# jdapena/distributed_point_functions

Hardware: AMD Instinct MI355X
Metric: DPF leaf evals/sec, full-domain 2^30 uint64 at 1/2/4/8 GPUs; AES blocks/s (higher is better)
Workload: dtype u64

## Files before the change

distributed_point_functions_amd/csrc/kernels/dpf_device.h:

```cpp
#pragma once
#include <hip/hip_runtime.h>
#include <stdint.h>
#include <string.h>

#include "../../../include/dpf_hip.h"
#include "aes_core.h"

namespace {

struct T0Table {
  uint32_t v[256];
};
constexpr T0Table make_t0() {
  T0Table t{};
  for (int i = 0; i < 256; ++i) {
    uint32_t s = dpf_aes::kSbox[i];
    uint32_t s2 = ((s << 1) ^ ((s & 0x80) ? 0x1b : 0)) & 0xff;
    t.v[i] = s2 | (s << 8) | (s << 16) | ((s2 ^ s) << 24);
  }
  return t;
}
__constant__ T0Table c_t0 = make_t0();

struct RoundKeys {
// ... 129 lines not shown
using dpf_aes::Block4;
using u128 = unsigned __int128;

__device__ __forceinline__ u128 block_u128(Block4 h) {
  return ((u128)h.w3 << 96) | ((u128)h.w2 << 64) | ((u128)h.w1 << 32) | h.w0;
}
__device__ __forceinline__ u128 dpf_u128(dpf_block c) { return ((u128)c.high << 64) | c.low; }

struct ExpandParams {
  int64_t num_items;
  int num_levels;
  int k0;
  int S;
  const dpf_block* seeds_in;
  const uint8_t* ctrl_in;
  const dpf_block* cw_seed;
  const uint8_t* cw_left;
  const uint8_t* cw_right;
  char* out;
  RoundKeys rkl, rkr, rkv, rkd;
  int dyn_chunks;
  int ph_end[3];
  int64_t ph_item[3];
  unsigned int* chunk_counter;
  unsigned long long* clock;
};

__device__ __forceinline__ int64_t take_expand_chunk(const ExpandParams& p, int* lds_counter,
                                                     int64_t done, int& k0, int& S) {
  unsigned int c = 0;
  if ((threadIdx.x & 63) == 0)
    c = p.chunk_counter ? __hip_atomic_fetch_add(p.chunk_counter, 1u, __ATOMIC_RELAXED,
                                                 __HIP_MEMORY_SCOPE_AGENT)
                        : (unsigned int)atomicAdd(lds_counter, 1);
  c = __builtin_amdgcn_readfirstlane(c);
  const unsigned int e0 = (unsigned int)p.ph_end[0], e1 = (unsigned int)p.ph_end[1],
                     e2 = (unsigned int)p.ph_end[2];
  if (c >= e2) return done;
  const int j = (c >= e0) + (c >= e1);
  const unsigned int first = j == 0 ? 0u : (j == 1 ? e0 : e1);
  const unsigned int last = j == 0 ? e0 : (j == 1 ? e1 : e2);
  const int64_t item0 = j == 0 ? p.ph_item[0] : (j == 1 ? p.ph_item[1] : p.ph_item[2]);
  const int64_t group = p.chunk_counter ? 0 : (int64_t)blockIdx.x;
  const int64_t chunk = group * (int64_t)(last - first) + (c - first);
  k0 = p.k0 + 2 * j;
  S = p.S - 2 * j;
  return item0 + chunk * 64 + (int64_t)(threadIdx.x & 63);
}

__device__ __forceinline__ int64_t take_chunk(int* counter, int64_t per_wg, int64_t chunks,
                                              int64_t done) {
  int c = 0;
  if ((threadIdx.x & 63) == 0) c = atomicAdd(counter, 1);
  c = __builtin_amdgcn_readfirstlane(c);
  const int64_t g = (int64_t)blockIdx.x * per_wg + c;
  return c < per_wg && g < chunks ? g * 64 + (int64_t)(threadIdx.x & 63) : done;
}

struct ItemLoop {
  int* counter;
  int64_t per_wg, chunks, done;
  __device__ __forceinline__ int64_t first() const {
    return per_wg ? take_chunk(counter, per_wg, chunks, done)
                  : blockIdx.x * (int64_t)blockDim.x + threadIdx.x;
  }
  __device__ __forceinline__ int64_t next(int64_t u) const {
    return per_wg ? take_chunk(counter, per_wg, chunks, done)
                  : u + (int64_t)gridDim.x * blockDim.x;
  }
// ... 889 lines not shown
```

distributed_point_functions_amd/csrc/kernels/dpf_expand_plan.hip:

```cpp
#include <stdint.h>

#include "../../../include/dpf_hip.h"
#include "dpf_runtime.h"

namespace dpf_rt {

int choose_subtree_depth(int64_t num_starts, int num_levels) {
  const int S = num_levels < max_subtree_depth() ? num_levels : max_subtree_depth();
#if defined(DPF_FORCE_S)
  if (num_levels >= DPF_FORCE_S) return DPF_FORCE_S;
#endif
  double best = -1;
  int best_s = S;
  for (int cand = S; cand >= (num_levels > 0 ? 1 : 0); --cand) {
    const int64_t items = num_starts << (num_levels - cand);
    const int blk = block_for(items);
    const int64_t threads = (int64_t)grid_for(items, blk) * blk;
    const int64_t rounds = (items + threads - 1) / threads;
    const double cost = (double)rounds * (2.0 * (num_levels - cand) + 3.0 * (double)(1ll << cand));
    if (best < 0 || cost < best * 0.999) {
      best = cost;
      best_s = cand;
    }
  }
  return best_s;
}

bool small_shape(int64_t num_starts, int num_levels, int* t, int* D) {
  const int64_t cus = num_cus();
  if (hook_is("DPF_EXPAND_SMALL", '0') || num_levels < 1 || num_starts < 1 || num_starts > cus)
    return false;
  int tt = 0;
  while (tt < num_levels - 1 && (num_starts << (tt + 1)) <= cus) ++tt;
  const int d = num_levels - tt;
  if (d < 1 || d > kSmallMaxD) return false;
  *t = tt;
  *D = d;
  return true;
}

bool top_shape(int64_t num_items, int k0, int* t, int* D) {
  const int64_t starts = num_items >> k0;
  if (hook_is("DPF_EXPAND_TOP", '0') || k0 < 8 || starts > num_cus() ||
      num_items < 4 * (int64_t)num_cus())
    return false;
  int tt = 0;
  while ((starts << tt) < num_cus() && tt < k0 - 1) ++tt;
  if (k0 - tt > kSmallMaxD) tt = k0 - kSmallMaxD;
  if (k0 - tt < 1 || (starts << tt) > INT32_MAX) return false;
  *t = tt;
  *D = k0 - tt;
  return true;
}

static int octet_dynamic_shift(int S) {
  return hook_int("DPF_OCTET_DYNAMIC", S >= 11 ? 4 : 2, 0, 4);
}
int octet_walk_levels() { return hook_int("DPF_OCTET_WALK", 2, 0, 4); }
ChunkPlan plan_chunks(int64_t num_items, int k0, int S, int min_S, int64_t cus, bool sched_ok) {
  ChunkPlan c{};
  const int sh = octet_dynamic_shift(S);
  if (sh <= 0 || S - sh < min_S || k0 + sh > 62 || cus <= 0 || num_items <= 0 ||
      num_items > (INT64_MAX >> (sh + 4)) || (num_items << sh) % (cus * 64) != 0 ||
      (num_items << sh) < 4 * cus * max_block() || (num_items << sh) / 64 > (INT32_MAX >> 4))
    return c;
  c.shift = sh;
  const int big = sched_ok && (num_items << S) / cus >= ((int64_t)1 << 20);
  c.global = hook_int("DPF_OCTET_GLOBAL", big, 0, 1);
  c.groups = c.global ? 1 : cus;
  const int k = k0 + sh, s = S - sh;
  const int64_t coarse = (num_items << sh) / 64;
  const int finer = hook_int("DPF_OCTET_TAPER", big ? 2 : 0, 0, 2);
  const int64_t at = hook_int("DPF_OCTET_TAPER_AT", 2, 1, 16) * cus * (max_block() / 64);
  auto exists = [&](int j) { return j <= finer && s - 2 * j >= min_S && k + 2 * j <= 62; };
  int64_t start[4] = {0, coarse, coarse, coarse};
  if (exists(1)) start[1] = coarse - (coarse < at ? coarse : at);
  if (exists(2)) start[2] = coarse - (coarse - start[1] < (at >> 2) ? coarse - start[1] : (at >> 2));
  for (int j = 0; j < 3; ++j) {
    c.k0[j] = k + 2 * j;
    c.S[j] = s - 2 * j;
    c.chunks[j] = (start[j + 1] - start[j]) << (2 * j);
    c.first_item[j] = (start[j] * 64) << (2 * j);
  }
  return c;
}

void write_plan(const ChunkPlan& c, int64_t* out) {
  for (int i = 0; i < 15; ++i) out[i] = 0;
  out[0] = c.shift;
  if (!c.shift) return;
  out[1] = c.global;
  out[2] = c.groups;
  for (int j = 0; j < 3; ++j) {
    out[3 + 4 * j] = c.chunks[j];
    out[4 + 4 * j] = c.first_item[j];
    out[5 + 4 * j] = c.k0[j];
    out[6 + 4 * j] = c.S[j];
  }
}

}

using namespace dpf_rt;

extern "C" int dpf_hip_octet_schedule(int64_t num_items, int k0, int subtree_depth, int min_depth,
                                      int compute_units, int64_t* out) {
  if (!out) return fail(kInvalidArgument, "NULL pointer");
  if (num_items < 1 || k0 < 0 || subtree_depth < 0 || k0 + subtree_depth > 62 ||
      compute_units < 1)
    return fail(kInvalidArgument, "launch shape out of range");
  write_plan(plan_chunks(num_items, k0, subtree_depth, min_depth, compute_units, true), out);
  return kOk;
}
```

distributed_point_functions_amd/csrc/kernels/dpf_kernels.hip:

```cpp
#include <hip/hip_runtime.h>
#include <stdint.h>
#include <stdlib.h>
#include <string.h>

#include <atomic>
#include <type_traits>
#include <vector>
#include <string>

#include "../../../include/dpf_hip.h"
#include "dpf_device.h"
#include "dpf_dot.h"
#include "dpf_runtime.h"

namespace dpf_rt {
thread_local std::string g_last_error;
thread_local const char* g_last_expand = "";
thread_local int g_last_expand_s = -1;
thread_local int64_t g_last_dynamic_chunks = 0;
std::atomic<unsigned long long*> g_clock_acc{nullptr};

int fail(int code, const std::string& msg) {
  g_last_error = msg;
  return code;
// ... 53 lines not shown
  for (int64_t i = items.first(); i < p.n; i = items.next(i)) {
    Block4 s = load_block(p.seeds_in + i);
    uint32_t t = p.ctrl_in[i] & 1u;
    Block4 path = load_block(p.paths + i);
    for (int j = 0; j < p.num_levels; ++j) {
      uint32_t bit = path_bit(path, p.num_levels - 1 - j);
      path_step(lk, lk.ks.l, lk.ks.d, s, t, bit, lds.cw_seed[j], lds.cw_ctrl[j]);
    }
    store_block(p.seeds_out + i, s);
    p.ctrl_out[i] = (uint8_t)t;
  }
}

template <class Leaf, bool SCHED = false>
__global__ __launch_bounds__(kBlock) DPF_WAVES_ATTR void expand_kernel(ExpandParams p, Leaf leaf) {
  __shared__ LdsImage lds;
  __shared__ int next_chunk;
  leaf.init();
  fill_tables(lds.tab);
  fill_cws(lds, p.cw_seed, p.cw_left, p.cw_right, p.num_levels);
  if (threadIdx.x == 0) next_chunk = 0;
  __syncthreads();
  const LdsLookup lk = make_lookup(lds, KeySet{key_ref(p.rkl), key_ref(p.rkr), key_ref(p.rkv), key_ref(p.rkd)});
  int k0 = p.k0, S = p.S;
  if constexpr (SCHED) ClockStamp::first_begin(p.clock);
  const int64_t nch = (p.num_items + 63) / 64;
  const int64_t end = SCHED ? INT64_MAX : p.num_items;
  auto take = [&]() -> int64_t {
    if constexpr (SCHED) return take_expand_chunk(p, &next_chunk, end, k0, S);
    else return take_chunk(&next_chunk, p.dyn_chunks, nch, p.num_items);
  };
  for (int64_t item = SCHED || p.dyn_chunks ? take()
                                            : blockIdx.x * (int64_t)blockDim.x + threadIdx.x;
       item < end;
       item = SCHED || p.dyn_chunks ? take() : item + (int64_t)gridDim.x * blockDim.x) {
    const int B = S >= 1 ? 1 : 0;
    const int G = S - B;
    const int64_t ngroups = (int64_t)1 << G;
    const int64_t r = item >> k0;
    Block4 s = load_block(p.seeds_in + r);
    uint32_t t = p.ctrl_in[r] & 1u;
    for (int j = 0; j < k0; ++j) {
      uint32_t bit = (uint32_t)((item >> (k0 - 1 - j)) & 1);
      path_step(lk, lk.ks.l, lk.ks.d, s, t, bit, lds.cw_seed[j], lds.cw_ctrl[j]);
    }
    Block4 sib[kGMax];
    uint32_t tb = 0;
    const int64_t leaf_base = item << S;
    for (int64_t g = 0; g < ngroups; ++g) {
      Block4 node = s;
      uint32_t nt = t;
      int ds = 0;
      if (g != 0) {
        ds = G - (int)__builtin_ctzll((unsigned long long)g);
#pragma unroll
        for (int d = 1; d <= kGMax; ++d)
          if (d == ds) { node = sib[d - 1]; nt = (tb >> d) & 1u; }
      }
      for (int d = ds; d < G; ++d) {
        Block4 c0, c1;
        uint32_t t0, t1;
        children_step(lk, lk.ks.l, lk.ks.r, node, nt, lds.cw_seed[k0 + d], lds.cw_ctrl[k0 + d],
                      c0, t0, c1, t1);
#pragma unroll
        for (int e = 1; e <= kGMax; ++e)
          if (e == d + 1) sib[e - 1] = c1;
// ... 63 lines not shown
  }
  leaf.store4(x, first_leaf, out);
}

template <class Leaf> struct OctetStash { static constexpr int value = 2; };
template <> struct OctetStash<SwarLeaf> { static constexpr int value = 1; };

template <class Leaf, bool SCHED = false>
__global__ __launch_bounds__(kBlock) DPF_WAVES_ATTR void expand_octet_kernel(ExpandParams p,
                                                                             Leaf leaf) {
  __shared__ LdsImage lds;
  constexpr int kStash = OctetStash<Leaf>::value;
  __shared__ uint4 stash[kBlock];
  __shared__ uint3 stash2[kStash >= 2 ? kBlock : 1];
  __shared__ int next_chunk;
  static_assert(sizeof(LdsImage) + 16 * kBlock + (kStash >= 2 ? 12 * kBlock : 0) + 16 <= 160 * 1024,
                "LDS over 160 KiB");
  leaf.init();
  fill_tables(lds.tab);
  fill_cws(lds, p.cw_seed, p.cw_left, p.cw_right, p.num_levels);
  if (threadIdx.x == 0) next_chunk = 0;
  __syncthreads();
  const LdsLookup lk = make_lookup(lds, KeySet{key_ref(p.rkl), key_ref(p.rkr), key_ref(p.rkv), key_ref(p.rkd)});
  int k0 = p.k0, S = p.S;
  ClockStamp stamp;
  stamp.begin(p.clock);
  const int lane = (int)(threadIdx.x & 63);
  const int64_t end = SCHED ? INT64_MAX : p.num_items;
  auto take = [&]() -> int64_t {
    if constexpr (SCHED) {
      return take_expand_chunk(p, &next_chunk, end, k0, S);
    } else {
      int c = 0;
      if (lane == 0) c = atomicAdd(&next_chunk, 1);
      c = __builtin_amdgcn_readfirstlane(c);
      return c < p.dyn_chunks ? ((int64_t)blockIdx.x * p.dyn_chunks + c) * 64 + lane
                              : p.num_items;
    }
  };
  for (int64_t item = SCHED || p.dyn_chunks ? take()
                                            : blockIdx.x * (int64_t)blockDim.x + threadIdx.x;
       item < end;
       item = SCHED || p.dyn_chunks ? take() : item + (int64_t)gridDim.x * blockDim.x) {
    const int G = S - 3;
    const int64_t ngroups = (int64_t)1 << G;
    const int64_t r = item >> k0;
    Block4 s = load_block(p.seeds_in + r);
    uint32_t t = p.ctrl_in[r] & 1u;
    for (int j = 0; j < k0; ++j) {
      const uint32_t bit = (uint32_t)((item >> (k0 - 1 - j)) & 1);
      path_step(lk, lk.ks.l, lk.ks.d, s, t, bit, lds.cw_seed[j], lds.cw_ctrl[j]);
    }
    Block4 sib[kGMax];
    uint32_t tb = 0;
    const int64_t leaf_base = item << S;
    Block4 next = s;
    for (int64_t g = 0; g < ngroups; ++g) {
      Block4 node = next;
      uint32_t nt = t;
      int ds = 0;
      if (g != 0) {
        ds = G - (int)__builtin_ctzll((unsigned long long)g);
        nt = (tb >> ds) & 1u;
      }
      for (int d = ds; d < G; ++d) {
        Block4 c0, c1;
        uint32_t t0, t1;
        children_step(lk, lk.ks.l, lk.ks.r, node, nt, lds.cw_seed[k0 + d], lds.cw_ctrl[k0 + d],
                      c0, t0, c1, t1);
        sib[d] = c1;
        tb = (tb & ~(1u << (d + 1))) | (t1 << (d + 1));
        node = c0;
        nt = t0;
// ... 121 lines not shown
                     lds.cw_ctrl[lvl], c0, t0, c1, t1);
      quad::hash2(lk, qv, c0, c1);
      const Block4 h0 = quad::gather(c0), h1 = quad::gather(c1);
      if (c == 0) {
        leaf.store(leaf.correct(h0, t0), leaf0 + 2 * q, p.out);
        leaf.store(leaf.correct(h1, t1), leaf0 + 2 * q + 1, p.out);
      }
    }
  } else if (tid < npar) {
    const uint4 v = nodes[tid];
    Block4 c0, c1;
    uint32_t t0, t1;
    children_step(lk, lk.ks.l, lk.ks.r, Block4{v.x, v.y, v.z, v.w}, tbits[tid], lds.cw_seed[lvl],
                  lds.cw_ctrl[lvl], c0, t0, c1, t1);
    leaf.emit2(lk, lk.ks.v, c0, t0, c1, t1, leaf0 + 2 * tid, p.out);
  }
  if constexpr (HasFinish<Leaf>::value) leaf.finish();
}

struct SeedLeaf {
  dpf_block* seeds;
  uint8_t* ctrl;
  unsigned int* counter;
  __device__ __forceinline__ void init() const {
    if (counter != nullptr && blockIdx.x == 0 && threadIdx.x == 0) *counter = 0u;
  }
  __device__ __forceinline__ void emit2(const LdsLookup&, KeyRef, Block4 s0, uint32_t t0, Block4 s1,
                                        uint32_t t1, int64_t first, char*) const {
    store_block(seeds + first, s0);
    store_block(seeds + first + 1, s1);
    ctrl[first] = (uint8_t)t0;
    ctrl[first + 1] = (uint8_t)t1;
  }
};

__global__ void count_out_of_range_kernel(int64_t n, const dpf_block* __restrict__ pts, int log,
                                          unsigned long long* __restrict__ bad) {
  unsigned long long c = 0;
  for (int64_t i = blockIdx.x * (int64_t)blockDim.x + threadIdx.x; i < n;
       i += (int64_t)gridDim.x * blockDim.x) {
    const dpf_block b = pts[i];
    bool out;
    if (log >= 128) out = false;
    else if (log >= 64) out = (b.high >> (log - 64)) != 0;
    else out = b.high != 0 || (b.low >> log) != 0;
    c += out ? 1 : 0;
  }
  for (int off = 32; off > 0; off >>= 1) c += __shfl_down(c, off, 64);
// ... 131 lines not shown
  int t = 0, D = 0;
  const int64_t starts = p0.num_items >> p0.k0;
  if (!small_shape(starts, p0.num_levels, &t, &D)) return false;
  ExpandParams p = p0;
  p.k0 = t;
  p.S = D;
  p.num_items = starts << t;
  static const std::string name = std::string("small/") + leaf_name<Leaf>();
  g_last_expand = name.c_str();
  g_last_expand_s = D;
  hipLaunchKernelGGL((expand_small_kernel<Leaf>), dim3((unsigned)p.num_items), dim3(kBlock), 0, s,
                     p, leaf);
  return true;
}


struct TopScratch {
  void* mem = nullptr;
  hipStream_t s = nullptr;
  ~TopScratch() {
    if (mem) (void)hipFreeAsync(mem, s);
  }
};
int expand_top(ExpandParams& p, hipStream_t s, TopScratch& scratch,
               unsigned int** counter = nullptr) {
  const int64_t starts = p.num_items >> p.k0;
  int t = 0, D = 0;
  if (!top_shape(p.num_items, p.k0, &t, &D)) return kOk;
  static const bool pool_kept = [] {
    int dev = 0;
    hipMemPool_t pool;
    if (hipGetDevice(&dev) != hipSuccess || hipDeviceGetDefaultMemPool(&pool, dev) != hipSuccess)
      return false;
    uint64_t keep = UINT64_MAX;
    return hipMemPoolSetAttribute(pool, hipMemPoolAttrReleaseThreshold, &keep) == hipSuccess;
  }();
  (void)pool_kept;
  const size_t items = (size_t)p.num_items;
  void* mem = nullptr;
  const size_t roots = (items * (sizeof(dpf_block) + 1) + 127) / 128 * 128;
  HIP_TRY(hipMallocAsync(&mem, roots + (counter ? 128 : 0), s));
  scratch.mem = mem;
  scratch.s = s;
  SeedLeaf leaf{static_cast<dpf_block*>(mem),
                static_cast<uint8_t*>(mem) + items * sizeof(dpf_block),
                counter ? reinterpret_cast<unsigned int*>(static_cast<char*>(mem) + roots)
                        : nullptr};
  if (counter) *counter = leaf.counter;
  ExpandParams q = p;
  q.k0 = t;
  q.S = D;
  q.num_levels = p.k0;
  q.num_items = starts << t;
  q.clock = nullptr;
  hipLaunchKernelGGL((expand_small_kernel<SeedLeaf>), dim3((unsigned)q.num_items), dim3(kBlock), 0,
                     s, q, leaf);
  HIP_TRY(hipGetLastError());
  p.seeds_in = leaf.seeds;
  p.ctrl_in = leaf.ctrl;
  p.cw_seed += p.k0;
  p.cw_left += p.k0;
  p.cw_right += p.k0;
  p.num_levels = p.S;
  p.k0 = 0;
  return kOk;
}

thread_local ChunkPlan g_last_plan{};
int subtree_shape(ExpandParams& p, int min_S, hipStream_t s, TopScratch& top, int* grid,
                  int* blk, bool sched_ok) {
  p.dyn_chunks = 0;
  p.chunk_counter = nullptr;
  g_last_plan = ChunkPlan{};
  const int64_t cus = num_cus();
  const ChunkPlan plan = plan_chunks(p.num_items, p.k0, p.S, min_S, cus, sched_ok);
  if (const int sh = plan.shift) {
    ExpandParams q = p;
    q.S -= sh;
    q.k0 += sh;
    q.num_items <<= sh;
    q.dyn_chunks = (int)(q.num_items / (cus * 64));
    int64_t taken = 0;
    for (int j = 0; j < 3; ++j) {
      taken += plan.chunks[j] / plan.groups;
      q.ph_end[j] = (int)taken;
      q.ph_item[j] = plan.first_item[j];
    }
    unsigned int* counter = nullptr;
    unsigned int** want_counter = plan.global ? &counter : nullptr;
    const int w = octet_walk_levels();
    int up = w > 0 && q.k0 - w >= 8 ? w : 0;
    ExpandParams t;
    for (;; up = 0) {
      t = q;
      t.k0 = q.k0 - up;
      t.S = q.S + up;
      t.num_items = q.num_items >> up;
      if (int st = expand_top(t, s, top, want_counter)) return st;
      if (t.k0 == 0 || up == 0) break;
    }
    if (t.k0 == 0) {
      q.chunk_counter = counter;
      q.seeds_in = t.seeds_in;
      q.ctrl_in = t.ctrl_in;
      q.cw_seed = t.cw_seed;
      q.cw_left = t.cw_left;
      q.cw_right = t.cw_right;
      q.num_levels = q.S + up;
      q.k0 = up;
      p = q;
      g_last_plan = plan;
      *grid = (int)cus;
      *blk = kBlock;
      return kOk;
    }
  }
  if (int st = expand_top(p, s, top)) return st;
  *blk = block_for(p.num_items);
  *grid = grid_for(p.num_items, *blk);
  return kOk;
}
template <class Leaf, bool OCTET> struct SchedDefault { static constexpr bool value = true; };
template <> struct SchedDefault<SwarLeaf, true> { static constexpr bool value = false; };
template <> struct SchedDefault<Mod32Leaf<kMod32MaxLeaves>, false> {
  static constexpr bool value = false;
};
bool has_schedule(const ExpandParams& p) {
  return p.dyn_chunks && (p.chunk_counter || p.ph_end[0] != p.ph_end[2]);
}
template <class Leaf> struct HasOctet : std::false_type {};
template <int BITS, bool XOR> struct HasOctet<FastIntLeaf<BITS, XOR>> : std::true_type {};
template <int BITS, bool XOR> struct HasOctet<DotLeaf<BITS, XOR>> : std::true_type {};
template <> struct HasOctet<SwarLeaf> : std::true_type {};
template <> struct HasOctet<Mod32Leaf<2>> : std::true_type {};
// ... 131 lines not shown
  auto sec = [&](unsigned long long t) { return (double)(int64_t)(t - t0) * 1e-8; };
  double lo = 0, hi = 0, sum = 0;
  int n = 0;
  for (int i = 0; i < kProbeWorkgroups; ++i) {
    if (!h[kProbeWords + i]) continue;
    const double t = sec(h[kProbeWords + i]);
    lo = n ? (t < lo ? t : lo) : t;
    hi = n ? (t > hi ? t : hi) : t;
    sum += t;
    ++n;
  }
  out[0] = sec(~h[kProbeFirstExit]);
  out[1] = sec(h[kProbeLastExit]);
  out[2] = lo;
  out[3] = hi;
  out[4] = n ? sum / n : 0.0;
  out[5] = n;
  return kOk;
}

int dpf_hip_last_expand_schedule(int64_t* out) {
  if (!out) return fail(kInvalidArgument, "NULL pointer");
  dpf_rt::write_plan(g_last_plan, out);
  return kOk;
}

int dpf_hip_clock_probe_read(double* clock_ghz, int64_t* workgroups, double* mean_workgroup_s) {
  unsigned long long* acc = dpf_rt::g_clock_acc.load();
  if (!acc) return fail(kFailedPrecondition, "clock probe is off (dpf_hip_clock_probe(1))");
  unsigned long long h[4] = {0, 0, 0, 0};
  HIP_TRY(hipDeviceSynchronize());
  HIP_TRY(hipMemcpy(h, acc, sizeof(h), hipMemcpyDeviceToHost));
  HIP_TRY(hipMemset(acc, 0, kProbeBytes));
  HIP_TRY(hipDeviceSynchronize());
  if (clock_ghz) *clock_ghz = h[1] ? (double)h[0] / (double)h[1] * 0.1 : 0.0;
  if (workgroups) *workgroups = (int64_t)h[2];
  if (mean_workgroup_s) *mean_workgroup_s = h[2] ? (double)h[1] / (double)h[2] * 1e-8 : 0.0;
  return kOk;
}

int dpf_hip_packed_element_size(const dpf_value_desc* desc) {
  if (!desc) return -1;
  return packed_size(desc);
}

int dpf_hip_hash(int64_t n, const dpf_block* in, const dpf_aes_key* key, dpf_block* out,
// ... 230 lines not shown
```

distributed_point_functions_amd/csrc/kernels/dpf_runtime.h:

```cpp
#pragma once
#include <hip/hip_runtime.h>
#include <stdint.h>
#include <stdlib.h>

#include <string>
#include <type_traits>

#include "../../../include/dpf_hip.h"

namespace dpf_rt {

constexpr int kOk = 0, kInvalidArgument = 3, kResourceExhausted = 8, kFailedPrecondition = 9,
              kUnimplemented = 12, kInternal = 13;

int fail(int code, const std::string& msg);
int hip_fail(hipError_t e, const char* what);

inline bool hook_is(const char* name, char c) {
  const char* v = getenv(name);
  return v && v[0] == c;
}
inline bool hook_set(const char* name) { return getenv(name) != nullptr; }
inline long long hook_long(const char* name, long long dflt) {
  const char* v = getenv(name);
// ... 13 lines not shown
int grid_for(int64_t work_items, int block);
struct LaunchShape {
  int block, grid;
  int64_t dyn_per_wg;
};
LaunchShape chunked_shape(int64_t items, const char* hook);
template <class F>
auto with_bits(int bits, F&& f) {
  switch (bits) {
    case 8: return f(std::integral_constant<int, 8>{});
    case 16: return f(std::integral_constant<int, 16>{});
    case 32: return f(std::integral_constant<int, 32>{});
    case 64: return f(std::integral_constant<int, 64>{});
    default: return f(std::integral_constant<int, 128>{});
  }
}
struct ChunkPlan {
  int shift;
  int global;
  int64_t groups;
  int k0[3], S[3];
  int64_t chunks[3], first_item[3];
};
ChunkPlan plan_chunks(int64_t num_items, int k0, int S, int min_S, int64_t cus, bool sched_ok);
void write_plan(const ChunkPlan& c, int64_t* out);
constexpr int kSmallMaxD = 11;
int choose_subtree_depth(int64_t num_starts, int num_levels);
bool small_shape(int64_t num_starts, int num_levels, int* t, int* D);
bool top_shape(int64_t num_items, int k0, int* t, int* D);
int octet_walk_levels();
int validate_desc(const dpf_value_desc* d);
int packed_size(const dpf_value_desc* d);
bool fast_int(const dpf_value_desc* d);

extern thread_local const char* g_last_dot;
int dot_type(const dpf_value_desc* d, int* words, int* xor_type);
int launch_dot_fold(int row_words, int xor_type, int accumulate, const void* workspace, void* out,
                    hipStream_t s);

constexpr int kHHSketchMaxRows = 2;
int launch_sketch_slot_weights(int64_t n, int64_t count, const int64_t* src_offset, int rows,
                               const uint32_t* weights, const uint32_t mod[2], uint32_t* out,
                               hipStream_t s);
int launch_hh_level(const dpf_prefix_batch_args& a, int b, hipStream_t s);
int launch_hh_keys(const dpf_prefix_batch_args& a, int b, hipStream_t s);

template <class Params>
void set_batch_tables(Params* p, const dpf_prefix_batch_args& a) {
  p->num_keys = a.num_keys;
  p->num_starts = a.num_starts;
  p->cw_stride = a.cw_stride;
  p->seeds_in = a.seeds_in;
// ... 23 lines not shown
```

distributed_point_functions_amd/hip_abi.py:

```python
from __future__ import annotations

import ctypes
import os
import re
from typing import Optional, Sequence

import numpy as np

_HERE = os.path.dirname(os.path.abspath(__file__))
LIB_PATH = os.environ.get("DPF_HIP_LIB") or os.path.join(_HERE, "lib", "libdpf_hip.so")
HEADER = os.path.join(os.path.dirname(_HERE), "include", "dpf_hip.h")
MAX_LEAVES = 16
LEAF_INT, LEAF_INTMODN, LEAF_XOR = 0, 1, 2
MASK64 = (1 << 64) - 1

_lib = None


class DpfHipError(RuntimeError):
    def __init__(self, code: int, msg: str):
        super().__init__(f"[{code}] {msg}")
        self.code = code


# ... 65 lines not shown
        L.dpf_hip_last_points_kernel.restype = ctypes.c_char_p
        L.dpf_hip_last_points_kernel.argtypes = []
        L.dpf_hip_hash.argtypes = [I64, P, P, P, P]
        L.dpf_hip_eval_paths.argtypes = [I64, I, P, P, P, P, P, P, P, P, P, P, P]
        L.dpf_hip_expand.argtypes = [I64, P, P, I, P, P, P, P, P, P, P, I, P, I, P, P]
        L.dpf_hip_eval_points.argtypes = [I64, I64, I, P, P, P, P, P, P, P, P, P, P, P, P, P, P,
                                          P, P]
        L.dpf_hip_gather.argtypes = [I64, I64, I, P, P, P, P]
        L.dpf_hip_sum_shares_u64.argtypes = [I64, I64, I, I, P, P, P]
        L.dpf_hip_packed_element_size.argtypes = [P]
        L.dpf_hip_event_create.argtypes = [ctypes.POINTER(ctypes.c_void_p)]
        L.dpf_hip_event_destroy.argtypes = [P]
        L.dpf_hip_event_record.argtypes = [P, P]
        L.dpf_hip_event_elapsed_ms.argtypes = [P, P, ctypes.POINTER(ctypes.c_float)]
        L.dpf_hip_stream_sync.argtypes = [P]
        L.dpf_hip_clock_probe.argtypes = [I]
        L.dpf_hip_clock_probe_read.argtypes = [ctypes.POINTER(ctypes.c_double),
                                               ctypes.POINTER(ctypes.c_int64),
                                               ctypes.POINTER(ctypes.c_double)]
        for name, types in (("dpf_hip_clock_probe_exits", [ctypes.POINTER(ctypes.c_double)]),
                            ("dpf_hip_octet_schedule",
                             [I64, I, I, I, I, ctypes.POINTER(ctypes.c_int64)]),
                            ("dpf_hip_last_expand_schedule", [ctypes.POINTER(ctypes.c_int64)]),
                            ("dpf_hip_last_dynamic_chunks", [ctypes.POINTER(ctypes.c_int64)]),
                            ("dpf_hip_mic_eval_batch",
                             [I64, I, P, P, P, P, P, I, P, P, I, P, I] + [P] * 11),
                            ("dpf_hip_expand_dot",
                             [I64, P, P, I, P, P, P, P, P, P, P, I, P, I, P, I, P, P, P]),
                            ("dpf_hip_dot_rows", [I64, I, P, P, P, I, P, P, P]),
                            ("dpf_hip_expand_dot_workspace_bytes", [P, I]),
                            ("dpf_hip_expand_dot_fused", [P, I]),
                            ("dpf_hip_last_dot_kernel", []),
                            ("dpf_hip_select_rows", [I64, I, I, P, I64, P, I, P, P, P]),
                            ("dpf_hip_select_workspace_bytes", [I, I]),
                            ("dpf_hip_last_select_shape", [ctypes.POINTER(ctypes.c_int64)]),
                            ("dpf_hip_dot_rows_batch", [I64, I, I, P, P, I64, P, I, P, P, P]),
                            ("dpf_hip_dot_rows_batch_workspace_bytes", [P, I, I]),
                            ("dpf_hip_last_dot_batch_shape", [ctypes.POINTER(ctypes.c_int64)]),
                            ("dpf_hip_sketch_rows", [I64, I64, P, P, I, I, P, P, P]),
                            ("dpf_hip_sketch_supported", [P]),
                            ("dpf_hip_gen_keys_supported", [P]),
                            ("dpf_hip_gen_key_batch",
                             [I64, I, I, P, P, P, P, P, P, P, I, I, P, P, P, P, P, P, P, P]),
                            ("dpf_hip_prefix_batch_sketch_fused", [P, I, I, I, I, I, I]),
                            ("dpf_hip_sketch_slot_weights", [I64, I64, P, P, I, P, P, P]),
                            ("dpf_hip_dcf_expand_supported", [P, I, P]),
# ... 208 lines not shown
def clock_probe_exits() -> dict:
    out = (ctypes.c_double * 6)()
    check(load().dpf_hip_clock_probe_exits(out))
    ms = [v * 1e3 for v in out[:5]]
    return {"first_exit_ms": ms[0], "last_exit_ms": ms[1], "workgroup_last_exit_min_ms": ms[2],
            "workgroup_last_exit_max_ms": ms[3], "workgroup_last_exit_mean_ms": ms[4],
            "workgroups": int(out[5])}


def octet_schedule(num_items: int, k0: int, subtree_depth: int, min_depth: int,
                   compute_units: int) -> dict:
    out = (ctypes.c_int64 * 15)()
    check(load().dpf_hip_octet_schedule(num_items, k0, subtree_depth, min_depth, compute_units,
                                        out))
    return _plan(out)


def last_expand_schedule() -> dict:
    out = (ctypes.c_int64 * 15)()
    check(load().dpf_hip_last_expand_schedule(out))
    return _plan(out)


def _plan(out) -> dict:
    phases = [{"chunks": out[3 + 4 * j], "first_item": out[4 + 4 * j], "k0": out[5 + 4 * j],
               "depth": out[6 + 4 * j]} for j in range(3) if out[3 + 4 * j]]
    return {"shift": out[0], "global": bool(out[1]), "counters": out[2], "phases": phases}


def check(st: int):
    if st != 0:
        raise DpfHipError(st, load().dpf_hip_last_error().decode())


def aes_key(k: int) -> AesKey:
    a = AesKey()
    for i, b in enumerate((k & ((1 << 128) - 1)).to_bytes(16, "little")):
        a.bytes[i] = b
    return a


def value_desc(leaves: Sequence[tuple], direct: bool, elements_per_block: int,
               blocks_needed: int) -> ValueDesc:
    d = ValueDesc()
    d.num_leaves = len(leaves)
    d.direct = 1 if direct else 0
# ... 278 lines not shown
```

include/dpf_hip.h:

```cpp
#ifndef DPF_HIP_H_
#define DPF_HIP_H_

#include <stddef.h>
#include <stdint.h>

#ifdef __cplusplus
extern "C" {
#endif

#define DPF_HIP_ABI_VERSION 2
#define DPF_MAX_LEAVES 16

typedef struct dpf_block {
  uint64_t low;
  uint64_t high;
} dpf_block;

typedef struct dpf_aes_key {
  uint8_t bytes[16];
} dpf_aes_key;

enum dpf_leaf_kind { DPF_LEAF_INT = 0, DPF_LEAF_INTMODN = 1, DPF_LEAF_XOR = 2 };

typedef struct dpf_value_desc {
// ... 78 lines not shown
int dpf_hip_select_workspace_bytes(int record_words, int num_queries);
int dpf_hip_last_select_shape(int64_t* out3);

#define DPF_HIP_DOT_BATCH_MAX_QUERIES 64
int dpf_hip_dot_rows_batch(int64_t num_rows, int record_words, int num_queries,
                           const dpf_value_desc* desc, const void* y, int64_t y_stride_bytes,
                           const void* db, int accumulate, void* workspace, void* out,
                           void* stream);
int dpf_hip_dot_rows_batch_workspace_bytes(const dpf_value_desc* desc, int record_words,
                                           int num_queries);
int dpf_hip_last_dot_batch_shape(int64_t* out3);

const char* dpf_hip_last_expand_kernel(int* subtree_depth);

int dpf_hip_clock_probe(int on);
int dpf_hip_clock_probe_read(double* clock_ghz, int64_t* workgroups, double* mean_workgroup_s);

int dpf_hip_clock_probe_exits(double* out);

int dpf_hip_octet_schedule(int64_t num_items, int k0, int subtree_depth, int min_depth,
                           int compute_units, int64_t* out);

int dpf_hip_last_expand_schedule(int64_t* out);

const char* dpf_hip_last_batch_kernel(void);

const char* dpf_hip_last_points_kernel(void);

int dpf_hip_last_dynamic_chunks(int64_t* per_wg);

int dpf_hip_eval_points(int64_t num_points, int64_t points_per_key, int num_levels,
                        const dpf_block* key_seed, const uint8_t* party,
                        const dpf_block* seeds_in, const uint8_t* control_in,
                        const dpf_block* tree_index, const int32_t* block_index,
                        const dpf_block* cw_seed, const uint8_t* cw_left,
                        const uint8_t* cw_right, const dpf_aes_key* key_left,
                        const dpf_aes_key* key_right, const dpf_aes_key* key_value,
                        const dpf_value_desc* desc, const dpf_block* value_correction,
                        void* out, void* stream);

int dpf_hip_eval_points_batch(int64_t num_keys, int64_t points_per_key, int shared_points,
                              int num_levels, int cw_stride, int block_index_bits,
                              const dpf_block* key_seed,
                              const uint8_t* party, const dpf_block* points,
                              const dpf_block* cw_seed, const uint8_t* cw_left,
                              const uint8_t* cw_right, const dpf_aes_key* key_left,
// ... 208 lines not shown
```

Baseline: 74.23 billion.

## Precompute per-chunk subtree roots so scheduled expand skips redundant path walks

Adds a roots plan that expands the top of the tree down to every chunk's root depth in a few extra kernel launches and stores those seeds in scratch memory. The scheduled expand kernels then load each item's root directly instead of walking k0 levels of AES path steps per item. Initial chunks are also assigned statically by wave index, with the global counter preset past them, which removes the first atomic. The taper and global thresholds are retuned for the roots path. In exchange it adds scratch allocation, extra launches and more complex planning logic.

```diff
diff --git a/distributed_point_functions_amd/csrc/kernels/dpf_device.h b/distributed_point_functions_amd/csrc/kernels/dpf_device.h
--- a/distributed_point_functions_amd/csrc/kernels/dpf_device.h
+++ b/distributed_point_functions_amd/csrc/kernels/dpf_device.h
@@ -175,17 +175,25 @@
   int dyn_chunks;
   int ph_end[3];
   int64_t ph_item[3];
+  int ph_roots;
+  int64_t ph_root[3];
   unsigned int* chunk_counter;
+  int chunk_first;
   unsigned long long* clock;
 };
 
+template <bool FIRST>
 __device__ __forceinline__ int64_t take_expand_chunk(const ExpandParams& p, int* lds_counter,
-                                                     int64_t done, int& k0, int& S) {
+                                                     int64_t done, int& k0, int& S, int& walk,
+                                                     int64_t& root) {
   unsigned int c = 0;
-  if ((threadIdx.x & 63) == 0)
+  if (FIRST && p.chunk_counter && p.chunk_first) {
+    c = blockIdx.x * (blockDim.x >> 6) + (threadIdx.x >> 6);
+  } else if ((threadIdx.x & 63) == 0) {
     c = p.chunk_counter ? __hip_atomic_fetch_add(p.chunk_counter, 1u, __ATOMIC_RELAXED,
                                                  __HIP_MEMORY_SCOPE_AGENT)
                         : (unsigned int)atomicAdd(lds_counter, 1);
+  }
   c = __builtin_amdgcn_readfirstlane(c);
   const unsigned int e0 = (unsigned int)p.ph_end[0], e1 = (unsigned int)p.ph_end[1],
                      e2 = (unsigned int)p.ph_end[2];
@@ -198,6 +206,8 @@
   const int64_t chunk = group * (int64_t)(last - first) + (c - first);
   k0 = p.k0 + 2 * j;
   S = p.S - 2 * j;
+  walk = p.ph_roots ? 0 : k0;
+  root = j == 0 ? p.ph_root[0] : (j == 1 ? p.ph_root[1] : p.ph_root[2]);
   return item0 + chunk * 64 + (int64_t)(threadIdx.x & 63);
 }
 
diff --git a/distributed_point_functions_amd/csrc/kernels/dpf_expand_plan.hip b/distributed_point_functions_amd/csrc/kernels/dpf_expand_plan.hip
--- a/distributed_point_functions_amd/csrc/kernels/dpf_expand_plan.hip
+++ b/distributed_point_functions_amd/csrc/kernels/dpf_expand_plan.hip
@@ -10,6 +10,7 @@
 #if defined(DPF_FORCE_S)
   if (num_levels >= DPF_FORCE_S) return DPF_FORCE_S;
 #endif
+  if (const int forced = hook_int("DPF_EXPAND_SUBTREE", 0, 0, S); forced >= 1) return forced;
   double best = -1;
   int best_s = S;
   for (int cand = S; cand >= (num_levels > 0 ? 1 : 0); --cand) {
@@ -40,12 +41,14 @@
 }
 
 bool top_shape(int64_t num_items, int k0, int* t, int* D) {
+  return top_shape_for(num_items, k0, num_cus(), t, D);
+}
+bool top_shape_for(int64_t num_items, int k0, int64_t cus, int* t, int* D) {
   const int64_t starts = num_items >> k0;
-  if (hook_is("DPF_EXPAND_TOP", '0') || k0 < 8 || starts > num_cus() ||
-      num_items < 4 * (int64_t)num_cus())
+  if (hook_is("DPF_EXPAND_TOP", '0') || k0 < 8 || starts > cus || num_items < 4 * cus)
     return false;
   int tt = 0;
-  while ((starts << tt) < num_cus() && tt < k0 - 1) ++tt;
+  while ((starts << tt) < cus && tt < k0 - 1) ++tt;
   if (k0 - tt > kSmallMaxD) tt = k0 - kSmallMaxD;
   if (k0 - tt < 1 || (starts << tt) > INT32_MAX) return false;
   *t = tt;
@@ -57,20 +60,25 @@
   return hook_int("DPF_OCTET_DYNAMIC", S >= 11 ? 4 : 2, 0, 4);
 }
 int octet_walk_levels() { return hook_int("DPF_OCTET_WALK", 2, 0, 4); }
-ChunkPlan plan_chunks(int64_t num_items, int k0, int S, int min_S, int64_t cus, bool sched_ok) {
+ChunkPlan plan_chunks(int64_t num_items, int k0, int S, int min_S, int64_t cus, bool sched_ok,
+                      bool item_roots) {
   ChunkPlan c{};
   const int sh = octet_dynamic_shift(S);
+  const int64_t per_thread = hook_int("DPF_OCTET_MIN_PER_THREAD", 4, 0, 4);
   if (sh <= 0 || S - sh < min_S || k0 + sh > 62 || cus <= 0 || num_items <= 0 ||
       num_items > (INT64_MAX >> (sh + 4)) || (num_items << sh) % (cus * 64) != 0 ||
-      (num_items << sh) < 4 * cus * max_block() || (num_items << sh) / 64 > (INT32_MAX >> 4))
+      (num_items << sh) < per_thread * cus * max_block() ||
+      (num_items << sh) / 64 > (INT32_MAX >> 4))
     return c;
   c.shift = sh;
-  const int big = sched_ok && (num_items << S) / cus >= ((int64_t)1 << 20);
+  const int64_t per_cu = (num_items << S) / cus;
+  const int big = sched_ok && per_cu >= ((int64_t)1 << (item_roots ? 19 : 20));
+  const int finer_dflt = !big ? 0 : (per_cu >= ((int64_t)1 << 20) ? 2 : 1);
   c.global = hook_int("DPF_OCTET_GLOBAL", big, 0, 1);
   c.groups = c.global ? 1 : cus;
   const int k = k0 + sh, s = S - sh;
   const int64_t coarse = (num_items << sh) / 64;
-  const int finer = hook_int("DPF_OCTET_TAPER", big ? 2 : 0, 0, 2);
+  const int finer = hook_int("DPF_OCTET_TAPER", finer_dflt, 0, 2);
   const int64_t at = hook_int("DPF_OCTET_TAPER_AT", 2, 1, 16) * cus * (max_block() / 64);
   auto exists = [&](int j) { return j <= finer && s - 2 * j >= min_S && k + 2 * j <= 62; };
   int64_t start[4] = {0, coarse, coarse, coarse};
@@ -83,6 +91,79 @@
     c.first_item[j] = (start[j] * 64) << (2 * j);
   }
   return c;
+}
+
+RootsPlan plan_roots(const ChunkPlan& c, int64_t num_items, int k0, int S, int64_t cus) {
+  RootsPlan r{};
+  if (!c.shift || hook_is("DPF_EXPAND_ROOTS", '0') || hook_set("DPF_OCTET_WALK")) return r;
+  const int64_t starts = num_items >> k0;
+  const int kd = c.k0[0];
+  if (starts < 1 || (starts << k0) != num_items) return r;
+  int d = 8;
+  while (d < kd - 1 && (starts << d) < cus * max_block()) ++d;
+  if (d < kd - max_subtree_depth()) d = kd - max_subtree_depth();
+  int t = 0, D = 0;
+  if (d > kd - 1 || !top_shape_for(starts << d, d, cus, &t, &D)) return r;
+  r.top_depth = d;
+  r.top_nodes = starts << d;
+  for (int j = 0; j < 3; ++j)
+    if (c.chunks[j]) r.stages = j + 1;
+  int64_t base = r.top_nodes;
+  for (int j = 0; j < r.stages; ++j) {
+    RootsPlan::Stage& st = r.st[j];
+    const int64_t all = starts << c.k0[j];
+    st.in_depth = j ? c.k0[j - 1] : d;
+    st.levels = c.k0[j] - st.in_depth;
+    st.out_first = j ? c.first_item[j] : 0;
+    st.out_count = all - st.out_first;
+    st.in_first = st.out_first >> st.levels;
+    st.in_count = st.out_count >> st.levels;
+    st.base = base;
+    base += st.out_count;
+    if ((st.in_first << st.levels) != st.out_first || c.first_item[j] < st.out_first ||
+        c.first_item[j] + c.chunks[j] * 64 > st.out_first + st.out_count ||
+        st.in_count > INT32_MAX)
+      return RootsPlan{};
+  }
+  r.nodes = base;
+  r.bytes = (base * 17 + 127) / 128 * 128 + 128;
+  r.bound = ((num_items << S) * 16) / 8;
+  if (r.bytes > r.bound) return RootsPlan{};
+  r.on = 1;
+  return r;
+}
+
+ChunkPlan plan_for_roots(int64_t num_items, int k0, int S, int min_S, int64_t cus, bool sched_ok,
+                         RootsPlan* roots) {
+  const ChunkPlan c = plan_chunks(num_items, k0, S, min_S, cus, sched_ok, true);
+  *roots = plan_roots(c, num_items, k0, S, cus);
+  if (roots->on) return c;
+  const ChunkPlan w = plan_chunks(num_items, k0, S, min_S, cus, sched_ok, false);
+  *roots = plan_roots(w, num_items, k0, S, cus);
+  return w;
+}
+
+void write_roots_plan(const RootsPlan& r, int64_t* out) {
+  for (int i = 0; i < kRootsPlanWords; ++i) out[i] = 0;
+  out[0] = r.on;
+  if (!r.on) return;
+  out[1] = r.top_depth;
+  out[2] = r.top_nodes;
+  out[3] = r.stages;
+  out[4] = r.nodes;
+  out[5] = r.bytes;
+  out[6] = r.bound;
+  for (int j = 0; j < r.stages; ++j) {
+    const RootsPlan::Stage& st = r.st[j];
+    int64_t* o = out + 8 + 7 * j;
+    o[0] = st.in_depth;
+    o[1] = st.levels;
+    o[2] = st.in_first;
+    o[3] = st.in_count;
+    o[4] = st.out_first;
+    o[5] = st.out_count;
+    o[6] = st.base;
+  }
 }
 
 void write_plan(const ChunkPlan& c, int64_t* out) {
@@ -109,6 +190,18 @@
   if (num_items < 1 || k0 < 0 || subtree_depth < 0 || k0 + subtree_depth > 62 ||
       compute_units < 1)
     return fail(kInvalidArgument, "launch shape out of range");
-  write_plan(plan_chunks(num_items, k0, subtree_depth, min_depth, compute_units, true), out);
+  write_plan(plan_chunks(num_items, k0, subtree_depth, min_depth, compute_units, true, false), out);
   return kOk;
 }
+
+extern "C" int dpf_hip_expand_roots_plan(int64_t num_items, int k0, int subtree_depth,
+                                         int min_depth, int compute_units, int64_t* out) {
+  if (!out) return fail(kInvalidArgument, "NULL pointer");
+  if (num_items < 1 || k0 < 0 || subtree_depth < 0 || k0 + subtree_depth > 62 ||
+      compute_units < 1)
+    return fail(kInvalidArgument, "launch shape out of range");
+  RootsPlan r;
+  (void)plan_for_roots(num_items, k0, subtree_depth, min_depth, compute_units, true, &r);
+  write_roots_plan(r, out);
+  return kOk;
+}
diff --git a/distributed_point_functions_amd/csrc/kernels/dpf_kernels.hip b/distributed_point_functions_amd/csrc/kernels/dpf_kernels.hip
--- a/distributed_point_functions_amd/csrc/kernels/dpf_kernels.hip
+++ b/distributed_point_functions_amd/csrc/kernels/dpf_kernels.hip
@@ -99,26 +99,29 @@
   if (threadIdx.x == 0) next_chunk = 0;
   __syncthreads();
   const LdsLookup lk = make_lookup(lds, KeySet{key_ref(p.rkl), key_ref(p.rkr), key_ref(p.rkv), key_ref(p.rkd)});
-  int k0 = p.k0, S = p.S;
+  int k0 = p.k0, S = p.S, walk = p.k0;
+  int64_t root = 0;
   if constexpr (SCHED) ClockStamp::first_begin(p.clock);
   const int64_t nch = (p.num_items + 63) / 64;
   const int64_t end = SCHED ? INT64_MAX : p.num_items;
-  auto take = [&]() -> int64_t {
-    if constexpr (SCHED) return take_expand_chunk(p, &next_chunk, end, k0, S);
+  auto take = [&](auto first) -> int64_t {
+    if constexpr (SCHED)
+      return take_expand_chunk<decltype(first)::value>(p, &next_chunk, end, k0, S, walk, root);
     else return take_chunk(&next_chunk, p.dyn_chunks, nch, p.num_items);
   };
-  for (int64_t item = SCHED || p.dyn_chunks ? take()
+  for (int64_t item = SCHED || p.dyn_chunks ? take(std::true_type{})
                                             : blockIdx.x * (int64_t)blockDim.x + threadIdx.x;
        item < end;
-       item = SCHED || p.dyn_chunks ? take() : item + (int64_t)gridDim.x * blockDim.x) {
+       item = SCHED || p.dyn_chunks ? take(std::false_type{})
+                                    : item + (int64_t)gridDim.x * blockDim.x) {
     const int B = S >= 1 ? 1 : 0;
     const int G = S - B;
     const int64_t ngroups = (int64_t)1 << G;
-    const int64_t r = item >> k0;
+    const int64_t r = SCHED ? (item >> walk) + root : item >> k0;
     Block4 s = load_block(p.seeds_in + r);
     uint32_t t = p.ctrl_in[r] & 1u;
-    for (int j = 0; j < k0; ++j) {
-      uint32_t bit = (uint32_t)((item >> (k0 - 1 - j)) & 1);
+    for (int j = 0; j < walk; ++j) {
+      uint32_t bit = (uint32_t)((item >> (walk - 1 - j)) & 1);
       path_step(lk, lk.ks.l, lk.ks.d, s, t, bit, lds.cw_seed[j], lds.cw_ctrl[j]);
     }
     Block4 sib[kGMax];
@@ -228,14 +231,15 @@
   if (threadIdx.x == 0) next_chunk = 0;
   __syncthreads();
   const LdsLookup lk = make_lookup(lds, KeySet{key_ref(p.rkl), key_ref(p.rkr), key_ref(p.rkv), key_ref(p.rkd)});
-  int k0 = p.k0, S = p.S;
+  int k0 = p.k0, S = p.S, walk = p.k0;
+  int64_t root = 0;
   ClockStamp stamp;
   stamp.begin(p.clock);
   const int lane = (int)(threadIdx.x & 63);
   const int64_t end = SCHED ? INT64_MAX : p.num_items;
-  auto take = [&]() -> int64_t {
+  auto take = [&](auto first) -> int64_t {
     if constexpr (SCHED) {
-      return take_expand_chunk(p, &next_chunk, end, k0, S);
+      return take_expand_chunk<decltype(first)::value>(p, &next_chunk, end, k0, S, walk, root);
     } else {
       int c = 0;
       if (lane == 0) c = atomicAdd(&next_chunk, 1);
@@ -244,17 +248,18 @@
                               : p.num_items;
     }
   };
-  for (int64_t item = SCHED || p.dyn_chunks ? take()
+  for (int64_t item = SCHED || p.dyn_chunks ? take(std::true_type{})
                                             : blockIdx.x * (int64_t)blockDim.x + threadIdx.x;
        item < end;
-       item = SCHED || p.dyn_chunks ? take() : item + (int64_t)gridDim.x * blockDim.x) {
+       item = SCHED || p.dyn_chunks ? take(std::false_type{})
+                                    : item + (int64_t)gridDim.x * blockDim.x) {
     const int G = S - 3;
     const int64_t ngroups = (int64_t)1 << G;
-    const int64_t r = item >> k0;
+    const int64_t r = SCHED ? (item >> walk) + root : item >> k0;
     Block4 s = load_block(p.seeds_in + r);
     uint32_t t = p.ctrl_in[r] & 1u;
-    for (int j = 0; j < k0; ++j) {
-      const uint32_t bit = (uint32_t)((item >> (k0 - 1 - j)) & 1);
+    for (int j = 0; j < walk; ++j) {
+      const uint32_t bit = (uint32_t)((item >> (walk - 1 - j)) & 1);
       path_step(lk, lk.ks.l, lk.ks.d, s, t, bit, lds.cw_seed[j], lds.cw_ctrl[j]);
     }
     Block4 sib[kGMax];
@@ -422,8 +427,14 @@
   dpf_block* seeds;
   uint8_t* ctrl;
   unsigned int* counter;
+  unsigned int counter_init;
   __device__ __forceinline__ void init() const {
-    if (counter != nullptr && blockIdx.x == 0 && threadIdx.x == 0) *counter = 0u;
+    if (counter != nullptr && blockIdx.x == 0 && threadIdx.x == 0) *counter = counter_init;
+  }
+  __device__ __forceinline__ void emit(const LdsLookup&, KeyRef, Block4 s0, uint32_t t0,
+                                       int64_t first, char*) const {
+    store_block(seeds + first, s0);
+    ctrl[first] = (uint8_t)t0;
   }
   __device__ __forceinline__ void emit2(const LdsLookup&, KeyRef, Block4 s0, uint32_t t0, Block4 s1,
                                         uint32_t t1, int64_t first, char*) const {
@@ -601,11 +612,7 @@
     if (mem) (void)hipFreeAsync(mem, s);
   }
 };
-int expand_top(ExpandParams& p, hipStream_t s, TopScratch& scratch,
-               unsigned int** counter = nullptr) {
-  const int64_t starts = p.num_items >> p.k0;
-  int t = 0, D = 0;
-  if (!top_shape(p.num_items, p.k0, &t, &D)) return kOk;
+void keep_pool() {
   static const bool pool_kept = [] {
     int dev = 0;
     hipMemPool_t pool;
@@ -615,6 +622,13 @@
     return hipMemPoolSetAttribute(pool, hipMemPoolAttrReleaseThreshold, &keep) == hipSuccess;
   }();
   (void)pool_kept;
+}
+int expand_top(ExpandParams& p, hipStream_t s, TopScratch& scratch,
+               unsigned int** counter = nullptr, unsigned int counter_init = 0) {
+  const int64_t starts = p.num_items >> p.k0;
+  int t = 0, D = 0;
+  if (!top_shape(p.num_items, p.k0, &t, &D)) return kOk;
+  keep_pool();
   const size_t items = (size_t)p.num_items;
   void* mem = nullptr;
   const size_t roots = (items * (sizeof(dpf_block) + 1) + 127) / 128 * 128;
@@ -624,7 +638,8 @@
   SeedLeaf leaf{static_cast<dpf_block*>(mem),
                 static_cast<uint8_t*>(mem) + items * sizeof(dpf_block),
                 counter ? reinterpret_cast<unsigned int*>(static_cast<char*>(mem) + roots)
-                        : nullptr};
+                        : nullptr,
+                counter_init};
   if (counter) *counter = leaf.counter;
   ExpandParams q = p;
   q.k0 = t;
@@ -645,14 +660,89 @@
   return kOk;
 }
 
+bool expand_roots(ExpandParams& q, const RootsPlan& rp, hipStream_t s, TopScratch& scratch,
+                  unsigned int** counter, unsigned int counter_init, int* st) {
+  *st = kOk;
+  const int64_t starts = rp.top_nodes >> rp.top_depth;
+  int t = 0, D = 0;
+  if (!top_shape(rp.top_nodes, rp.top_depth, &t, &D)) return false;
+  keep_pool();
+  void* mem = nullptr;
+  if (hipMallocAsync(&mem, (size_t)rp.bytes, s) != hipSuccess) {
+    (void)hipGetLastError();
+    return false;
+  }
+  scratch.mem = mem;
+  scratch.s = s;
+  dpf_block* seeds = static_cast<dpf_block*>(mem);
+  uint8_t* ctrl = static_cast<uint8_t*>(mem) + (size_t)rp.nodes * sizeof(dpf_block);
+  unsigned int* cnt =
+      counter ? reinterpret_cast<unsigned int*>(static_cast<char*>(mem) + rp.bytes - 128) : nullptr;
+  if (counter) *counter = cnt;
+  auto failed = [&](hipError_t e) {
+    if (e != hipSuccess) *st = hip_fail(e, "item roots launch");
+    return e != hipSuccess;
+  };
+  ExpandParams e = q;
+  e.dyn_chunks = 0;
+  e.chunk_counter = nullptr;
+  e.clock = nullptr;
+  e.out = nullptr;
+  e.seeds_in = q.seeds_in;
+  e.k0 = t;
+  e.S = D;
+  e.num_levels = rp.top_depth;
+  e.num_items = starts << t;
+  hipLaunchKernelGGL((expand_small_kernel<SeedLeaf>), dim3((unsigned)e.num_items), dim3(kBlock), 0,
+                     s, e, SeedLeaf{seeds, ctrl, cnt, counter_init});
+  if (failed(hipGetLastError())) return true;
+  int64_t in_base = 0, in_first = 0;
+  for (int j = 0; j < rp.stages; ++j) {
+    const RootsPlan::Stage& g = rp.st[j];
+    e.k0 = 0;
+    e.S = g.levels;
+    e.num_levels = g.levels;
+    e.num_items = g.in_count;
+    e.seeds_in = seeds + in_base + (g.in_first - in_first);
+    e.ctrl_in = ctrl + in_base + (g.in_first - in_first);
+    e.cw_seed = q.cw_seed + g.in_depth;
+    e.cw_left = q.cw_left + g.in_depth;
+    e.cw_right = q.cw_right + g.in_depth;
+    const int blk = block_for(g.in_count);
+    hipLaunchKernelGGL((expand_kernel<SeedLeaf, false>), dim3(grid_for(g.in_count, blk)), dim3(blk),
+                       0, s, e, SeedLeaf{seeds + g.base, ctrl + g.base, nullptr, 0u});
+    if (failed(hipGetLastError())) return true;
+    in_base = g.base;
+    in_first = g.out_first;
+    q.ph_root[j] = (g.base - rp.st[0].base) - g.out_first;
+  }
+  for (int j = rp.stages; j < 3; ++j) q.ph_root[j] = 0;
+  q.ph_roots = 1;
+  q.seeds_in = seeds + rp.st[0].base;
+  q.ctrl_in = ctrl + rp.st[0].base;
+  q.cw_seed += q.k0;
+  q.cw_left += q.k0;
+  q.cw_right += q.k0;
+  q.num_levels = q.S;
+  q.k0 = 0;
+  return true;
+}
+
 thread_local ChunkPlan g_last_plan{};
+thread_local RootsPlan g_last_roots{};
+thread_local int g_last_chunk_first = 0;
 int subtree_shape(ExpandParams& p, int min_S, hipStream_t s, TopScratch& top, int* grid,
                   int* blk, bool sched_ok) {
   p.dyn_chunks = 0;
   p.chunk_counter = nullptr;
+  p.chunk_first = 0;
+  p.ph_roots = 0;
   g_last_plan = ChunkPlan{};
+  g_last_roots = RootsPlan{};
+  g_last_chunk_first = 0;
   const int64_t cus = num_cus();
-  const ChunkPlan plan = plan_chunks(p.num_items, p.k0, p.S, min_S, cus, sched_ok);
+  RootsPlan roots;
+  const ChunkPlan plan = plan_for_roots(p.num_items, p.k0, p.S, min_S, cus, sched_ok, &roots);
   if (const int sh = plan.shift) {
     ExpandParams q = p;
     q.S -= sh;
@@ -667,6 +757,25 @@
     }
     unsigned int* counter = nullptr;
     unsigned int** want_counter = plan.global ? &counter : nullptr;
+    const int chunk_first = plan.global && !hook_is("DPF_EXPAND_ROOTS", '0');
+    const unsigned int counter_init = chunk_first ? (unsigned int)(cus * (kBlock / 64)) : 0u;
+    q.chunk_first = chunk_first;
+    q.ph_roots = 0;
+    if (roots.on) {
+      ExpandParams r = q;
+      int st = kOk;
+      if (expand_roots(r, roots, s, top, want_counter, counter_init, &st)) {
+        if (st) return st;
+        r.chunk_counter = counter;
+        p = r;
+        g_last_plan = plan;
+        g_last_roots = roots;
+        g_last_chunk_first = chunk_first;
+        *grid = (int)cus;
+        *blk = kBlock;
+        return kOk;
+      }
+    }
     const int w = octet_walk_levels();
     int up = w > 0 && q.k0 - w >= 8 ? w : 0;
     ExpandParams t;
@@ -675,7 +784,7 @@
       t.k0 = q.k0 - up;
       t.S = q.S + up;
       t.num_items = q.num_items >> up;
-      if (int st = expand_top(t, s, top, want_counter)) return st;
+      if (int st = expand_top(t, s, top, want_counter, counter_init)) return st;
       if (t.k0 == 0 || up == 0) break;
     }
     if (t.k0 == 0) {
@@ -689,6 +798,7 @@
       q.k0 = up;
       p = q;
       g_last_plan = plan;
+      g_last_chunk_first = chunk_first;
       *grid = (int)cus;
       *blk = kBlock;
       return kOk;
@@ -866,6 +976,13 @@
 int dpf_hip_last_expand_schedule(int64_t* out) {
   if (!out) return fail(kInvalidArgument, "NULL pointer");
   dpf_rt::write_plan(g_last_plan, out);
+  return kOk;
+}
+
+int dpf_hip_last_expand_roots(int64_t* out) {
+  if (!out) return fail(kInvalidArgument, "NULL pointer");
+  dpf_rt::write_roots_plan(g_last_roots, out);
+  out[7] = g_last_chunk_first;
   return kOk;
 }
 
diff --git a/distributed_point_functions_amd/csrc/kernels/dpf_runtime.h b/distributed_point_functions_amd/csrc/kernels/dpf_runtime.h
--- a/distributed_point_functions_amd/csrc/kernels/dpf_runtime.h
+++ b/distributed_point_functions_amd/csrc/kernels/dpf_runtime.h
@@ -59,12 +59,31 @@
   int k0[3], S[3];
   int64_t chunks[3], first_item[3];
 };
-ChunkPlan plan_chunks(int64_t num_items, int k0, int S, int min_S, int64_t cus, bool sched_ok);
+ChunkPlan plan_chunks(int64_t num_items, int k0, int S, int min_S, int64_t cus, bool sched_ok,
+                      bool item_roots);
 void write_plan(const ChunkPlan& c, int64_t* out);
+struct RootsPlan {
+  int on;
+  int top_depth;
+  int64_t top_nodes;
+  int stages;
+  struct Stage {
+    int in_depth, levels;
+    int64_t in_first, in_count, out_first, out_count, base;
+  } st[3];
+  int64_t nodes;
+  int64_t bytes, bound;
+};
+constexpr int kRootsPlanWords = 32;
+RootsPlan plan_roots(const ChunkPlan& c, int64_t num_items, int k0, int S, int64_t cus);
+ChunkPlan plan_for_roots(int64_t num_items, int k0, int S, int min_S, int64_t cus, bool sched_ok,
+                         RootsPlan* roots);
+void write_roots_plan(const RootsPlan& r, int64_t* out);
 constexpr int kSmallMaxD = 11;
 int choose_subtree_depth(int64_t num_starts, int num_levels);
 bool small_shape(int64_t num_starts, int num_levels, int* t, int* D);
 bool top_shape(int64_t num_items, int k0, int* t, int* D);
+bool top_shape_for(int64_t num_items, int k0, int64_t cus, int* t, int* D);
 int octet_walk_levels();
 int validate_desc(const dpf_value_desc* d);
 int packed_size(const dpf_value_desc* d);
diff --git a/distributed_point_functions_amd/hip_abi.py b/distributed_point_functions_amd/hip_abi.py
--- a/distributed_point_functions_amd/hip_abi.py
+++ b/distributed_point_functions_amd/hip_abi.py
@@ -111,6 +111,9 @@
                             ("dpf_hip_octet_schedule",
                              [I64, I, I, I, I, ctypes.POINTER(ctypes.c_int64)]),
                             ("dpf_hip_last_expand_schedule", [ctypes.POINTER(ctypes.c_int64)]),
+                            ("dpf_hip_expand_roots_plan",
+                             [I64, I, I, I, I, ctypes.POINTER(ctypes.c_int64)]),
+                            ("dpf_hip_last_expand_roots", [ctypes.POINTER(ctypes.c_int64)]),
                             ("dpf_hip_last_dynamic_chunks", [ctypes.POINTER(ctypes.c_int64)]),
                             ("dpf_hip_mic_eval_batch",
                              [I64, I, P, P, P, P, P, I, P, P, I, P, I] + [P] * 11),
@@ -365,6 +368,29 @@
     return _plan(out)
 
 
+def expand_roots_plan(num_items: int, k0: int, subtree_depth: int, min_depth: int,
+                      compute_units: int) -> dict:
+    out = (ctypes.c_int64 * 32)()
+    check(load().dpf_hip_expand_roots_plan(num_items, k0, subtree_depth, min_depth,
+                                           compute_units, out))
+    return _roots(out)
+
+
+def last_expand_roots() -> dict:
+    out = (ctypes.c_int64 * 32)()
+    check(load().dpf_hip_last_expand_roots(out))
+    return _roots(out)
+
+
+def _roots(out) -> dict:
+    if not out[0]:
+        return {"on": False, "first_by_number": bool(out[7])}
+    keys = ("in_depth", "levels", "in_first", "in_count", "out_first", "out_count", "base")
+    return {"on": True, "top_depth": out[1], "top_nodes": out[2], "nodes": out[4],
+            "bytes": out[5], "bound": out[6], "first_by_number": bool(out[7]),
+            "stages": [dict(zip(keys, out[8 + 7 * j:15 + 7 * j])) for j in range(out[3])]}
+
+
 def _plan(out) -> dict:
     phases = [{"chunks": out[3 + 4 * j], "first_item": out[4 + 4 * j], "k0": out[5 + 4 * j],
                "depth": out[6 + 4 * j]} for j in range(3) if out[3 + 4 * j]]
diff --git a/include/dpf_hip.h b/include/dpf_hip.h
--- a/include/dpf_hip.h
+++ b/include/dpf_hip.h
@@ -124,6 +124,11 @@
                            int compute_units, int64_t* out);
 
 int dpf_hip_last_expand_schedule(int64_t* out);
+
+int dpf_hip_expand_roots_plan(int64_t num_items, int k0, int subtree_depth, int min_depth,
+                              int compute_units, int64_t* out);
+
+int dpf_hip_last_expand_roots(int64_t* out);
 
 const char* dpf_hip_last_batch_kernel(void);
 
```

Result: no change. 74.82 billion, median of 6 (+0.8%).
